# cwida/ALP

Measured on AMD Instinct MI355X. Metric: ALP fused decode (falp + patch) throughput, decoded doubles, higher is better.
Workload: dtype f64

## Files before the change

### alp_amd/csrc/init_kernels.hip

```cpp
#include <cstdlib>

#include "launch.hpp"
#include "rd_dictionary_order.hpp"
#include "search_device.hpp"

namespace alpgpu {

constexpr int kMaxSampledVectors = 9;
constexpr int kInitThreads       = 64 * kMaxSampledVectors;
#ifndef ALPGPU_INIT_ASYNC_WAVES
#define ALPGPU_INIT_ASYNC_WAVES 4
#endif
constexpr int kInitAsyncWaves        = ALPGPU_INIT_ASYNC_WAVES;
#ifndef ALPGPU_INIT_ASYNC_OCC
#define ALPGPU_INIT_ASYNC_OCC (ALPGPU_INIT_ASYNC_WAVES == 4 ? 5 : 8)
#endif
constexpr int kInitAsyncWavesPerSimd = ALPGPU_INIT_ASYNC_OCC;

__device__ __forceinline__ int wave_scan_max_i32(int v) {
	int t;
	t = __builtin_amdgcn_update_dpp(-1, v, 0x111, 0xf, 0xf, false), v = t > v ? t : v;
	t = __builtin_amdgcn_update_dpp(-1, v, 0x112, 0xf, 0xf, false), v = t > v ? t : v;
	t = __builtin_amdgcn_update_dpp(-1, v, 0x114, 0xf, 0xf, false), v = t > v ? t : v;
	t = __builtin_amdgcn_update_dpp(-1, v, 0x118, 0xf, 0xf, false), v = t > v ? t : v;
	t = __builtin_amdgcn_update_dpp(-1, v, 0x142, 0xa, 0xf, false), v = t > v ? t : v;
	t = __builtin_amdgcn_update_dpp(-1, v, 0x143, 0xc, 0xf, false), v = t > v ? t : v;
	return v;
}

constexpr int kMaxSamples = kMaxSampledVectors * 32;

struct __attribute__((aligned(16))) RdWaveScratch {
	uint32_t len[kMaxSamples];
	uint32_t hist[kMaxSamples + 8];
};

__device__ __forceinline__ uint32_t rd_left_of(uint32_t composite, int cut) { return (composite >> 16) >> (16 - cut); }

__device__ __forceinline__ void rd_build_runs(RdWaveScratch& W, uint32_t* first, const uint32_t* s_key, int n_smp, int cut, int lane) {
	for (int b = 0; b < kMaxSamples + 8; b += 64) {
		const int j = b + lane;
		if (j < kMaxSamples) {
			W.len[j] = 0u;
			if (first) { first[j] = 0xFFFFFFFFu; }
		}
		if (j < kMaxSamples + 8) { W.hist[j] = 0u; }
	}
	wave_lds_sync();
	int carry = 0;
	for (int b = 0; b < n_smp; b += 64) {
		const int      j     = b + lane;
		const bool     valid = j < n_smp;
		const uint32_t left  = valid ? rd_left_of(s_key[j], cut) : 0u;
		const uint32_t prev  = (valid && j > 0) ? rd_left_of(s_key[j - 1], cut) : ~left;
		const bool     head  = valid && (j == 0 || left != prev);
		int            st    = wave_scan_max_i32(head ? j : -1);
		st                   = st < 0 ? carry : st;
		if (valid) {
			atomicAdd(&W.len[st], 1u);
			if (first) { atomicMin(&first[st], s_key[j] & 0xFFFFu); }
		}
		carry = __builtin_amdgcn_readlane(st, 63);
	}
	wave_lds_sync();
}

template <bool ASYNC>
__device__ __forceinline__ void store_rowgroup_state(alpgpu_rowgroup_state* __restrict__ dst, const alpgpu_rowgroup_state& st) {
	if constexpr (!ASYNC) {
		*dst = st;
	} else {
		uint64_t w[4];
		__builtin_memcpy(w, &st, 32);
		w[1] = (w[1] & 0x00FFFFFFFFFFFFFFull) | (static_cast<uint64_t>(kStateReady) << 56);
		uint64_t* d64 = reinterpret_cast<uint64_t*>(dst);
		__hip_atomic_store(d64 + 0, w[0], __ATOMIC_RELAXED, __HIP_MEMORY_SCOPE_AGENT);
		__hip_atomic_store(d64 + 2, w[2], __ATOMIC_RELAXED, __HIP_MEMORY_SCOPE_AGENT);
		__hip_atomic_store(d64 + 3, w[3], __ATOMIC_RELAXED, __HIP_MEMORY_SCOPE_AGENT);
		asm volatile("s_waitcnt vmcnt(0)" ::: "memory");
		__hip_atomic_store(d64 + 1, w[1], __ATOMIC_RELAXED, __HIP_MEMORY_SCOPE_AGENT);
	}
}

constexpr int kInitAsyncTileWaves = 8;
template <bool ASYNC, int W, int BITS>
constexpr int init_waves_per_simd() {
	return !ASYNC ? 1 : (W == kInitAsyncWaves ? kInitAsyncWavesPerSimd : (W == kInitAsyncTileWaves ? (BITS == 32 ? 8 : 6) : 1));
}
template <class P, bool FROM_SAMPLES, int W, bool ASYNC>
__global__ __launch_bounds__(64 * W, (init_waves_per_simd<ASYNC, W, P::kBits>())) void k_rowgroup_init(const typename P::value_t* __restrict__ in, uint64_t n_vectors,
                                                          alpgpu_rowgroup_state* __restrict__ rgs, int force_rd,
                                                          uint16_t* __restrict__ rd_order, uint64_t rg_first, uint64_t rg_end, double* __restrict__ cut_est_out,
                                                          uint32_t adaptive_base) {
	static_assert(!ASYNC || !FROM_SAMPLES, "the persistent form gathers its own samples");
	static_assert(W >= 2 && W <= kMaxSampledVectors, "the scratch arrays are sized for 9 wavefronts; wavefront 0 and the order replay use two of them");
	__shared__ typename P::value_t smp[kMaxSampledVectors * 32];
	__shared__ uint32_t best_key[kMaxSampledVectors];
	__shared__ uint32_t      s_key[kMaxSamples];
	constexpr int kRdScratch = W > 4 ? W : 4;
#ifdef ALPGPU_EXPERIMENT_INIT_SMALL_LDS
	__shared__ RdWaveScratch s_rd[1];
#else
	__shared__ RdWaveScratch s_rd[kRdScratch];
#endif
	__shared__ uint32_t      s_first[kMaxSamples];
	__shared__ double        s_cut_est[17];
	__shared__ uint8_t       s_cut_ds[17];
	__shared__ int           s_best_cut;
	__shared__ int           s_scheme;
	__shared__ alpgpu_rowgroup_state s_state;

	const int      lane    = lane_id();
	const int      wave    = wave_in_wg();
	const int      tid     = static_cast<int>(threadIdx.x);
	(void)rg_end;
	uint32_t walkers = gridDim.x;
	if constexpr (ASYNC) {
		if (adaptive_base != 0 && adaptive_base < gridDim.x) {
			const bool     rd    = rgs[4 * lane].scheme == ALPGPU_SCHEME_ALP_RD;
			const bool     heavy = __builtin_popcountll(ballot64(rd)) >= 32;
			walkers              = heavy ? gridDim.x : adaptive_base;
			if (blockIdx.x >= walkers) { return; }
		}
	}
	for (uint64_t rg = rg_first + blockIdx.x; ASYNC ? rg < rg_end : rg == rg_first + blockIdx.x; rg += ASYNC ? walkers : 1u << 30) {
	if (ASYNC) { __syncthreads(); }
	int n_sv, n_smp, samples_size;
	if constexpr (FROM_SAMPLES) {
		n_smp        = static_cast<int>(n_vectors);
		n_sv         = (n_smp + 31) / 32;
		samples_size = n_smp < 32 ? n_smp : 32;
		for (int sv = wave; sv < n_sv; sv += W) {
			if (lane < 32) { smp[sv * 32 + lane] = in[288ull * blockIdx.x + sv * samples_size + (lane < samples_size ? lane : 0)]; }
		}
	} else {
		const uint64_t v_first = rg * kRowgroup;
		const int      nv      = static_cast<int>((n_vectors - v_first) < kRowgroup ? (n_vectors - v_first) : kRowgroup);
		n_sv                   = (nv + 11) / 12;
		n_smp                  = 32 * n_sv;
		samples_size           = 32;
		for (int sv = wave; sv < n_sv; sv += W) {
			if (lane < 32) { smp[sv * 32 + lane] = in[(v_first + 12ull * sv) * kVec + 32ull * lane]; }
		}
	}
	if (tid < kMaxSampledVectors) { best_key[tid] = 0xFFFFFFFFu; }
	__syncthreads();

	if (!force_rd) {
		constexpr int  kTail       = P::kNumCombos % 64;
		constexpr bool kTailOnSide = P::kBits == 32 && kTail > 0 && kTail <= 2;
		constexpr int  kRounds     = kTailOnSide ? P::kNumCombos / 64 : (P::kNumCombos + 63) / 64;
		constexpr int  kItemsPerSv = kRounds + (kTailOnSide ? 1 : 0);
#pragma unroll 1
		for (int item = wave; item < n_sv * kItemsPerSv; item += W) {
			const int sv = item / kItemsPerSv;
			const int r  = item - sv * kItemsPerSv;
			uint32_t  my_key = 0xFFFFFFFFu;
			if (kTailOnSide && r == kRounds) {
				const int  half   = lane >> 5, sidx = lane & 31;
				const int  c      = P::kNumCombos - kTail + (half < kTail ? half : 0);
				const bool active = half < kTail && sidx < samples_size;
				const typename P::Coef k = P::coef(P::combos().e[c], P::combos().f[c]);
				const float   v  = static_cast<float>(smp[sv * 32 + (sidx < samples_size ? sidx : 0)]);
				const int32_t q  = encode_value_f32(v, k.exp10, k.frac_f);
				const bool    ok = active & (decode_value_f32(q, k.fact, k.frac_e) == v);
				const uint64_t bal     = ballot64(ok);
				const int      non_exc = __builtin_popcount(static_cast<uint32_t>(half ? (bal >> 32) : bal));
				int32_t        mx = ok ? q : INT32_MIN, mn = ok ? q : INT32_MAX;
#define ALPGPU_MINMAX_STEP(CTRL, ROWS)                                                                                  \
	{                                                                                                                   \
		const int32_t omx = __builtin_amdgcn_update_dpp(mx, mx, CTRL, ROWS, 0xf, false);                                \
		const int32_t omn = __builtin_amdgcn_update_dpp(mn, mn, CTRL, ROWS, 0xf, false);                                \
		mx                = omx > mx ? omx : mx;                                                                        \
		mn                = omn < mn ? omn : mn;                                                                        \
	}
				ALPGPU_MINMAX_STEP(0x111, 0xf)
				ALPGPU_MINMAX_STEP(0x112, 0xf)
				ALPGPU_MINMAX_STEP(0x114, 0xf)
				ALPGPU_MINMAX_STEP(0x118, 0xf)
				ALPGPU_MINMAX_STEP(0x142, 0xa)
#undef ALPGPU_MINMAX_STEP
				if (sidx == 31 && half < kTail && non_exc >= 2) {
					const uint32_t size = static_cast<uint32_t>(samples_size) * static_cast<uint32_t>(P::bits(mx, mn)) +
					                      static_cast<uint32_t>(samples_size - non_exc) * (P::kExcBits + 16u);
					my_key              = (size << 8) | static_cast<uint32_t>(c);
				}
			} else {
				const int c = lane + 64 * r;
				if (c < P::kNumCombos) {
					const typename P::Coef k = P::coef(P::combos().e[c], P::combos().f[c]);
					typename P::Acc        acc;
					P::start(acc);
					if constexpr (P::kBits == 64) {
						int s = 0;
						for (; s + 4 <= samples_size; s += 4) {
							P::step(acc, smp[sv * 32 + s], k);
							P::step(acc, smp[sv * 32 + s + 1], k);
							P::step(acc, smp[sv * 32 + s + 2], k);
							P::step(acc, smp[sv * 32 + s + 3], k);
						}
						for (; s < samples_size; ++s) { P::step(acc, smp[sv * 32 + s], k); }
					} else {
#pragma unroll 4
						for (int s = 0; s < samples_size; ++s) { P::step(acc, smp[sv * 32 + s], k); }
					}
					P::finish(acc);
					const int     non_exc = acc.non_exc;
					const int64_t mx = acc.mx, mn = acc.mn;
					if (non_exc >= 2) {
						const uint32_t size = static_cast<uint32_t>(samples_size) * static_cast<uint32_t>(P::bits(mx, mn)) +
						                      static_cast<uint32_t>(samples_size - non_exc) * (P::kExcBits + 16u);
						my_key              = (size << 8) | static_cast<uint32_t>(c);
					}
				}
			}
			my_key = wave_min_u32(my_key);
			if (lane == 0 && my_key != 0xFFFFFFFFu) { atomicMin(&best_key[sv], my_key); }
		}
	}
	__syncthreads();

	if (tid == 0) {
		uint32_t best_size = static_cast<uint32_t>(samples_size) * (P::kExcBits + 16u) + static_cast<uint32_t>(samples_size) * P::kExcBits;
		int      ce[kMaxSampledVectors], cf[kMaxSampledVectors], cn[kMaxSampledVectors];
		int      n_c = 0;
		for (int w = 0; w < n_sv; ++w) {
			int e = 0, f = 0;
			if (best_key[w] != 0xFFFFFFFFu) {
				const int      c    = static_cast<int>(best_key[w] & 0xFFu);
				const uint32_t size = best_key[w] >> 8;
				e                   = P::combos().e[c];
				f                   = P::combos().f[c];
				best_size           = size < best_size ? size : best_size;
			}
			int hit = -1;
			for (int i = 0; i < n_c; ++i) {
				if (ce[i] == e && cf[i] == f) { hit = i; }
			}
			if (hit < 0) {
				ce[n_c] = e, cf[n_c] = f, cn[n_c] = 1;
				++n_c;
			} else {
				++cn[hit];
			}
		}
		alpgpu_rowgroup_state st;
		st.k = 0;
		for (int i = 0; i < 10; ++i) { st.combos[i] = 0; }
		st.rd_rbw = st.rd_lbw = st.rd_dict_size = st.pad = 0;
		for (int i = 0; i < 8; ++i) { st.rd_dict[i] = 0; }
		if (force_rd || best_size >= P::kRdThreshold) {
			st.scheme = ALPGPU_SCHEME_ALP_RD;
		} else {
			st.scheme = ALPGPU_SCHEME_ALP;
			for (int i = 1; i < n_c; ++i) {
				const int e = ce[i], f = cf[i], n = cn[i];
				int       j = i - 1;
				while (j >= 0 && (n > cn[j] || (n == cn[j] && e > ce[j]) || (n == cn[j] && e == ce[j] && f > cf[j]))) {
					ce[j + 1] = ce[j], cf[j + 1] = cf[j], cn[j + 1] = cn[j];
					--j;
				}
				ce[j + 1] = e, cf[j + 1] = f, cn[j + 1] = n;
			}
			const int k = n_c < 5 ? n_c : 5;
			st.k        = static_cast<uint8_t>(k);
#pragma unroll
			for (int i = 0; i < 5; ++i) {
				st.combos[2 * i]     = i < k ? static_cast<uint8_t>(ce[i]) : 0;
				st.combos[2 * i + 1] = i < k ? static_cast<uint8_t>(cf[i]) : 0;
			}
		}
		s_scheme = st.scheme;
		if (st.scheme != ALPGPU_SCHEME_ALP_RD) {
			store_rowgroup_state<ASYNC>(rgs + rg, st);
			if (rd_order) { rd_order[rg * ALPGPU_RD_ORDER_STRIDE] = 0; }
		} else {
			s_state = st;
		}
	}
	__syncthreads();
	if (s_scheme != ALPGPU_SCHEME_ALP_RD) { continue; }
#ifdef ALPGPU_EXPERIMENT_INIT_SMALL_LDS
	continue;
#endif

	uint32_t* s_unsorted = reinterpret_cast<uint32_t*>(&s_rd[0]);
	static_assert(sizeof(RdWaveScratch) >= kMaxSamples * sizeof(uint32_t), "scratch reuse");
	static_assert(kMaxSamples % 4 == 0, "the rank loop reads four keys at a time");
	constexpr int kSortSlots = (kMaxSamples + 64 * W - 1) / (64 * W);
	for (int t = tid; t < kMaxSamples; t += 64 * W) {
		uint32_t c = 0xFFFFFFFFu;
		if (t < n_smp) { c = (static_cast<uint32_t>(P::pattern(smp[32 * (t / samples_size) + (t % samples_size)]) >> (P::kBits - 16)) << 16) | static_cast<uint32_t>(t); }
		s_unsorted[t] = c;
	}
	__syncthreads();
	uint32_t my_key[kSortSlots];
	int      my_rank[kSortSlots];
#pragma unroll
	for (int u = 0; u < kSortSlots; ++u) {
		const int t = tid + u * 64 * W;
		my_key[u]   = 0;
		my_rank[u]  = 0;
		if (t < n_smp) {
			my_key[u]          = s_unsorted[t];
			const u32x4* quads = reinterpret_cast<const u32x4*>(s_unsorted);
			const int    n_q   = (n_smp + 3) / 4;
			for (int q = 0; q < n_q; ++q) {
				const u32x4 k = quads[q];
				my_rank[u] += (k[0] < my_key[u] ? 1 : 0) + (k[1] < my_key[u] ? 1 : 0) + (k[2] < my_key[u] ? 1 : 0) + (k[3] < my_key[u] ? 1 : 0);
			}
		}
	}
	__syncthreads();
#pragma unroll
	for (int u = 0; u < kSortSlots; ++u) {
		if (tid + u * 64 * W < n_smp) { s_key[my_rank[u]] = my_key[u]; }
	}
	__syncthreads();

#ifdef ALPGPU_EXPERIMENT_RD_STOP_AFTER_SORT
	continue;
#endif
	RdWaveScratch& WS = s_rd[wave];
#ifdef ALPGPU_EXPERIMENT_RD_ONE_CUT
	const int forced_cut = 12;
#else
	const int forced_cut = (force_rd & 0x100) ? (force_rd & 0xFF) : 0;
#endif
	for (int cut = wave + 1; cut <= 16; cut += W) {
		const int rbw = P::kBits - cut;
		if (forced_cut != 0 && cut != forced_cut) {
			if (lane == 0) {
				s_cut_est[cut] = 1.7976931348623157e308;
				s_cut_ds[cut]  = 0;
			}
			continue;
		}
		rd_build_runs(WS, nullptr, s_key, n_smp, cut, lane);
		int distinct = 0;
		for (int b = 0; b < n_smp; b += 64) {
			const int      j = b + lane;
			const uint32_t L = j < n_smp ? WS.len[j] : 0u;
			if (L) { atomicAdd(&WS.hist[L], 1u); }
			distinct += __builtin_popcountll(__ballot(L != 0));
		}
		wave_lds_sync();
		uint32_t covered = 0;
		int      taken   = 0;
		for (int top = n_smp; top >= 1 && taken < 8; top -= 64) {
			const int      cval = top - lane;
			const uint32_t h    = cval >= 1 ? WS.hist[cval] : 0u;
			const uint32_t inc    = wave_scan_add_u32(h);
			const uint32_t before = static_cast<uint32_t>(taken) + inc - h;
			const uint32_t after  = static_cast<uint32_t>(taken) + inc;
			const uint32_t mine   = (after < 8u ? after : 8u) - (before < 8u ? before : 8u);
			const uint32_t part   = wave_scan_add_u32(mine * static_cast<uint32_t>(cval > 0 ? cval : 0));
			covered += static_cast<uint32_t>(__builtin_amdgcn_readlane(static_cast<int>(part), 63));
			taken += __builtin_amdgcn_readlane(static_cast<int>(inc), 63);
		}
		const uint32_t excs = static_cast<uint32_t>(n_smp) - covered;
		const int      ds   = distinct < 8 ? distinct : 8;
		const int      lbw  = ds <= 2 ? 1 : (ds <= 4 ? 2 : 3);
		if (lane == 0) {
			s_cut_est[cut] = static_cast<double>(rbw + lbw) + static_cast<double>(excs * 32u) / static_cast<double>(n_smp);
			s_cut_ds[cut]  = static_cast<uint8_t>(ds);
		}
		wave_lds_sync();
	}
	__syncthreads();
	if (tid == 0) {
		double best = 1.7976931348623157e308;
		int    bc   = 1;
		for (int cut = 1; cut <= 16; ++cut) {
			if (s_cut_est[cut] < best) {
				best = s_cut_est[cut];
				bc   = cut;
			}
		}
		s_best_cut = bc;
		if (cut_est_out != nullptr) { cut_est_out[blockIdx.x] = best; }
	}
	__syncthreads();
	if (wave == 0) {
		static_assert(sizeof(RdOrderLds) <= (kRdScratch - 1) * sizeof(RdWaveScratch), "order replay arrays alias s_rd[1..]");
		RdOrderLds& s_order = *reinterpret_cast<RdOrderLds*>(&s_rd[1]);
		const int best_cut = s_best_cut;
		const int rbw      = P::kBits - best_cut;
		const int ds       = s_cut_ds[best_cut];
		rd_build_runs(WS, s_first, s_key, n_smp, best_cut, lane);
		int distinct = 0;
		for (int b = 0; b < n_smp; b += 64) {
			const int      j    = b + lane;
			const bool     head = j < n_smp && WS.len[j] != 0;
			const uint64_t hb   = __ballot(head);
			if (head) { s_order.sorted[distinct + __builtin_popcountll(hb & ((1ull << lane) - 1ull))] = s_first[j]; }
			distinct += __builtin_popcountll(hb);
		}
		wave_lds_sync();
		for (int b = 0; b < n_smp; b += 64) {
			const int      j   = b + lane;
			const uint32_t L   = j < n_smp ? WS.len[j] : 0u;
			const uint32_t fo  = j < n_smp ? s_first[j] : 0u;
			int            ord = 0;
			for (int g = 0; g < distinct; ++g) { ord += s_order.sorted[g] < fo ? 1 : 0; }
			if (L != 0) {
				s_order.okey[ord] = rd_left_of(s_key[j], best_cut);
				s_order.ocnt[ord] = L;
			}
		}
		wave_lds_sync();
#ifndef ALPGPU_EXPERIMENT_SKIP_RD_ORDER
		if (lane == 0) { rd_reference_order(s_order, distinct); }
#endif
		wave_lds_sync();
		if (rd_order) {
			uint16_t* o = rd_order + rg * ALPGPU_RD_ORDER_STRIDE;
			for (int i = lane; i < distinct; i += 64) { o[1 + i] = static_cast<uint16_t>(s_order.sorted[i] & 0xFFFFu); }
			if (lane == 0) { o[0] = static_cast<uint16_t>(distinct); }
		}
		if constexpr (ASYNC) {
			if (rd_order) {
				__builtin_amdgcn_fence(__ATOMIC_RELEASE, "agent");
				asm volatile("s_waitcnt vmcnt(0)" ::: "memory");
			}
		}
		if (lane == 0) {
			const int             lbw = ds <= 2 ? 1 : (ds <= 4 ? 2 : 3);
			alpgpu_rowgroup_state st  = s_state;
			st.rd_rbw                 = static_cast<uint8_t>(rbw);
			st.rd_lbw                 = static_cast<uint8_t>(lbw);
			st.rd_dict_size           = static_cast<uint8_t>(ds);
#pragma unroll
			for (int i = 0; i < 8; ++i) { st.rd_dict[i] = i < ds ? static_cast<uint16_t>(s_order.sorted[i] & 0xFFFFu) : 0; }
			store_rowgroup_state<ASYNC>(rgs + rg, st);
		}
	}
	}
}

int launch_rowgroup_init(hipStream_t stream, const double* d_in, uint64_t n_vectors, alpgpu_rowgroup_state* d_rgs, uint16_t* d_rd_order, uint64_t rg_first,
                         uint64_t rg_count) {
	const uint64_t n_rg = (n_vectors + kRowgroup - 1) / kRowgroup;
	if (rg_first >= n_rg) { return ALPGPU_OK; }
	if (rg_count == 0 || rg_first + rg_count > n_rg) { rg_count = n_rg - rg_first; }
	hipLaunchKernelGGL((k_rowgroup_init<PrecF64, false, kMaxSampledVectors, false>), dim3(static_cast<unsigned>(rg_count)), dim3(kInitThreads), 0, stream, d_in,
	                   n_vectors, d_rgs, 0, d_rd_order, rg_first, rg_first + rg_count, static_cast<double*>(nullptr), 0u);
	return hipGetLastError() == hipSuccess ? ALPGPU_OK : ALPGPU_ERR_HIP;
}

template <class P>
static int launch_rowgroup_init_async_t(hipStream_t stream, const typename P::value_t* d_in, uint64_t n_vectors, alpgpu_rowgroup_state* d_rgs, uint16_t* d_rd_order,
                                        uint64_t rg_first, uint64_t rg_count, int grid, bool tile_shaped, uint32_t adaptive_base = 0) {
	if (rg_count == 0) { return ALPGPU_OK; }
	const uint64_t g = rg_count < static_cast<uint64_t>(grid) ? rg_count : static_cast<uint64_t>(grid);
	if (g == rg_count) {
		hipLaunchKernelGGL((k_rowgroup_init<P, false, kMaxSampledVectors, true>), dim3(static_cast<unsigned>(g)), dim3(kInitThreads), 0, stream, d_in, n_vectors, d_rgs, 0,
		                   d_rd_order, rg_first, rg_first + rg_count, static_cast<double*>(nullptr), 0u);
	} else if (tile_shaped) {
		hipLaunchKernelGGL((k_rowgroup_init<P, false, kInitAsyncTileWaves, true>), dim3(static_cast<unsigned>(g)), dim3(64 * kInitAsyncTileWaves), 0, stream, d_in, n_vectors,
		                   d_rgs, 0, d_rd_order, rg_first, rg_first + rg_count, static_cast<double*>(nullptr), adaptive_base);
	} else {
		hipLaunchKernelGGL((k_rowgroup_init<P, false, kInitAsyncWaves, true>), dim3(static_cast<unsigned>(g)), dim3(64 * kInitAsyncWaves), 0, stream, d_in, n_vectors, d_rgs,
		                   0, d_rd_order, rg_first, rg_first + rg_count, static_cast<double*>(nullptr), adaptive_base);
	}
	return hipGetLastError() == hipSuccess ? ALPGPU_OK : ALPGPU_ERR_HIP;
}
int launch_rowgroup_init_async(hipStream_t stream, const double* d_in, uint64_t n_vectors, alpgpu_rowgroup_state* d_rgs, uint16_t* d_rd_order, uint64_t rg_first,
                               uint64_t rg_count, int grid, bool tile_shaped, uint32_t adaptive_base) {
	return launch_rowgroup_init_async_t<PrecF64>(stream, d_in, n_vectors, d_rgs, d_rd_order, rg_first, rg_count, grid, tile_shaped, adaptive_base);
}
int launch_rowgroup_init_async_f32(hipStream_t stream, const float* d_in, uint64_t n_vectors, alpgpu_rowgroup_state* d_rgs, uint16_t* d_rd_order, uint64_t rg_first,
                                   uint64_t rg_count, int grid) {
	static const bool tile = std::getenv("ALPGPU_F32_SEARCH_TILE") != nullptr;
	return launch_rowgroup_init_async_t<PrecF32>(stream, d_in, n_vectors, d_rgs, d_rd_order, rg_first, rg_count, grid, tile);
}

int launch_state_from_samples(hipStream_t stream, const double* d_samples, uint32_t n_samples, alpgpu_rowgroup_state* d_state, int force_rd, double* d_cut_estimate) {
	hipLaunchKernelGGL((k_rowgroup_init<PrecF64, true, kMaxSampledVectors, false>), dim3(1), dim3(kInitThreads), 0, stream, d_samples, static_cast<uint64_t>(n_samples),
	                   d_state, force_rd, static_cast<uint16_t*>(nullptr), 0ull, 1ull, d_cut_estimate, 0u);
	return hipGetLastError() == hipSuccess ? ALPGPU_OK : ALPGPU_ERR_HIP;
}

int launch_rowgroup_init_f32(hipStream_t stream, const float* d_in, uint64_t n_vectors, alpgpu_rowgroup_state* d_rgs, uint16_t* d_rd_order,
                             uint64_t rg_first, uint64_t rg_count) {
	const uint64_t n_rg = (n_vectors + kRowgroup - 1) / kRowgroup;
	if (rg_first >= n_rg) { return ALPGPU_OK; }
	if (rg_count == 0 || rg_first + rg_count > n_rg) { rg_count = n_rg - rg_first; }
	hipLaunchKernelGGL((k_rowgroup_init<PrecF32, false, kMaxSampledVectors, false>), dim3(static_cast<unsigned>(rg_count)), dim3(kInitThreads), 0, stream, d_in,
	                   n_vectors, d_rgs, 0, d_rd_order, rg_first, rg_first + rg_count, static_cast<double*>(nullptr), 0u);
	return hipGetLastError() == hipSuccess ? ALPGPU_OK : ALPGPU_ERR_HIP;
}

int launch_state_from_samples_f32(hipStream_t stream, const float* d_samples, uint32_t n_samples, alpgpu_rowgroup_state* d_state, int force_rd, double* d_cut_estimate) {
	hipLaunchKernelGGL((k_rowgroup_init<PrecF32, true, kMaxSampledVectors, false>), dim3(1), dim3(kInitThreads), 0, stream, d_samples, static_cast<uint64_t>(n_samples),
	                   d_state, force_rd, static_cast<uint16_t*>(nullptr), 0ull, 1ull, d_cut_estimate, 0u);
	return hipGetLastError() == hipSuccess ? ALPGPU_OK : ALPGPU_ERR_HIP;
}

}
```

Before: 4461.

## Compute ALP-RD run lengths in registers via ballots instead of LDS atomics

Replaces the per-wave LDS scratch (run lengths plus histogram built with LDS atomics) with register-resident sorted keys and ballot bitmasks that give run heads and lengths directly. The top-8 coverage is found by eight wave-wide max reductions instead of a histogram scan. The dictionary-order replay now scatters first-occurrence indices instead of doing an O(distinct) rank loop per lane. LDS use shrinks to a union, which could allow higher occupancy in the init kernel. This is an init-path change whose effect on the fused decode metric may be small. The rewritten first-occurrence and order logic risks subtle correctness differences.

```diff
diff --git a/alp_amd/csrc/init_kernels.hip b/alp_amd/csrc/init_kernels.hip
--- a/alp_amd/csrc/init_kernels.hip
+++ b/alp_amd/csrc/init_kernels.hip
@@ -30,39 +30,62 @@
 
 constexpr int kMaxSamples = kMaxSampledVectors * 32;
 
-struct __attribute__((aligned(16))) RdWaveScratch {
-	uint32_t len[kMaxSamples];
-	uint32_t hist[kMaxSamples + 8];
+__device__ __forceinline__ uint32_t rd_left_of(uint32_t composite, int cut) { return (composite >> 16) >> (16 - cut); }
+
+constexpr int kKeyChunks = (kMaxSamples + 63) / 64;
+struct RdSortedKeys {
+	uint32_t key[kKeyChunks], prev[kKeyChunks];
 };
-
-__device__ __forceinline__ uint32_t rd_left_of(uint32_t composite, int cut) { return (composite >> 16) >> (16 - cut); }
-
-__device__ __forceinline__ void rd_build_runs(RdWaveScratch& W, uint32_t* first, const uint32_t* s_key, int n_smp, int cut, int lane) {
-	for (int b = 0; b < kMaxSamples + 8; b += 64) {
-		const int j = b + lane;
-		if (j < kMaxSamples) {
-			W.len[j] = 0u;
-			if (first) { first[j] = 0xFFFFFFFFu; }
-		}
-		if (j < kMaxSamples + 8) { W.hist[j] = 0u; }
-	}
-	wave_lds_sync();
-	int carry = 0;
-	for (int b = 0; b < n_smp; b += 64) {
-		const int      j     = b + lane;
-		const bool     valid = j < n_smp;
-		const uint32_t left  = valid ? rd_left_of(s_key[j], cut) : 0u;
-		const uint32_t prev  = (valid && j > 0) ? rd_left_of(s_key[j - 1], cut) : ~left;
-		const bool     head  = valid && (j == 0 || left != prev);
-		int            st    = wave_scan_max_i32(head ? j : -1);
-		st                   = st < 0 ? carry : st;
-		if (valid) {
-			atomicAdd(&W.len[st], 1u);
-			if (first) { atomicMin(&first[st], s_key[j] & 0xFFFFu); }
-		}
-		carry = __builtin_amdgcn_readlane(st, 63);
-	}
-	wave_lds_sync();
+__device__ __forceinline__ void rd_load_keys(RdSortedKeys& K, const uint32_t* s_key, int n_smp, int lane) {
+#pragma unroll
+	for (int c = 0; c < kKeyChunks; ++c) {
+		const int j = 64 * c + lane;
+		K.key[c]    = j < n_smp ? s_key[j] : 0xFFFFFFFFu;
+		K.prev[c]   = (j > 0 && j < n_smp) ? s_key[j - 1] : 0u;
+	}
+}
+
+struct RdRuns {
+	uint64_t head[kKeyChunks];
+	uint32_t len[kKeyChunks];
+	int      distinct;
+};
+__device__ __forceinline__ void rd_runs(RdRuns& R, const RdSortedKeys& K, int n_smp, int cut, int lane) {
+	R.distinct = 0;
+#pragma unroll
+	for (int c = 0; c < kKeyChunks; ++c) {
+		const int j = 64 * c + lane;
+		R.head[c]   = ballot64((j < n_smp) & ((j == 0) | (rd_left_of(K.key[c], cut) != rd_left_of(K.prev[c], cut))));
+		R.distinct += __builtin_popcountll(R.head[c]);
+	}
+	int next_start = n_smp;
+#pragma unroll
+	for (int c = kKeyChunks - 1; c >= 0; --c) {
+		const uint64_t above = R.head[c] & ~((2ull << lane) - 1ull);
+		const int      next  = above ? 64 * c + __builtin_ctzll(above) : next_start;
+		R.len[c]             = ((R.head[c] >> lane) & 1ull) ? static_cast<uint32_t>(next - (64 * c + lane)) : 0u;
+		if (R.head[c]) { next_start = 64 * c + __builtin_ctzll(R.head[c]); }
+	}
+}
+
+__device__ __forceinline__ uint32_t rd_top8_mass(const RdRuns& R, int n_smp, int lane) {
+	if (R.distinct <= 8) { return static_cast<uint32_t>(n_smp); }
+	static_assert(kMaxSamples < 512, "positions take 9 bits");
+	uint32_t u[kKeyChunks];
+#pragma unroll
+	for (int c = 0; c < kKeyChunks; ++c) { u[c] = R.len[c] ? (R.len[c] << 9) | static_cast<uint32_t>(64 * c + lane) : 0u; }
+	uint32_t covered = 0;
+#pragma unroll
+	for (int i = 0; i < 8; ++i) {
+		uint32_t m = u[0];
+#pragma unroll
+		for (int c = 1; c < kKeyChunks; ++c) { m = u[c] > m ? u[c] : m; }
+		const uint32_t top = static_cast<uint32_t>(__builtin_amdgcn_readlane(wave_scan_max_i32(static_cast<int>(m)), 63));
+		covered += top >> 9;
+#pragma unroll
+		for (int c = 0; c < kKeyChunks; ++c) { u[c] = u[c] == top ? 0u : u[c]; }
+	}
+	return covered;
 }
 
 template <bool ASYNC>
@@ -93,16 +116,14 @@
                                                           uint16_t* __restrict__ rd_order, uint64_t rg_first, uint64_t rg_end, double* __restrict__ cut_est_out,
                                                           uint32_t adaptive_base) {
 	static_assert(!ASYNC || !FROM_SAMPLES, "the persistent form gathers its own samples");
-	static_assert(W >= 2 && W <= kMaxSampledVectors, "the scratch arrays are sized for 9 wavefronts; wavefront 0 and the order replay use two of them");
+	static_assert(W >= 2 && W <= kMaxSampledVectors, "best_key and the sample arrays are sized for 9 sampled vectors");
 	__shared__ typename P::value_t smp[kMaxSampledVectors * 32];
 	__shared__ uint32_t best_key[kMaxSampledVectors];
 	__shared__ uint32_t      s_key[kMaxSamples];
-	constexpr int kRdScratch = W > 4 ? W : 4;
-#ifdef ALPGPU_EXPERIMENT_INIT_SMALL_LDS
-	__shared__ RdWaveScratch s_rd[1];
-#else
-	__shared__ RdWaveScratch s_rd[kRdScratch];
-#endif
+	__shared__ union {
+		uint32_t   unsorted[kMaxSamples];
+		RdOrderLds order;
+	} s_rdx;
 	__shared__ uint32_t      s_first[kMaxSamples];
 	__shared__ double        s_cut_est[17];
 	__shared__ uint8_t       s_cut_ds[17];
@@ -280,12 +301,8 @@
 	}
 	__syncthreads();
 	if (s_scheme != ALPGPU_SCHEME_ALP_RD) { continue; }
-#ifdef ALPGPU_EXPERIMENT_INIT_SMALL_LDS
-	continue;
-#endif
-
-	uint32_t* s_unsorted = reinterpret_cast<uint32_t*>(&s_rd[0]);
-	static_assert(sizeof(RdWaveScratch) >= kMaxSamples * sizeof(uint32_t), "scratch reuse");
+
+	uint32_t* s_unsorted = s_rdx.unsorted;
 	static_assert(kMaxSamples % 4 == 0, "the rank loop reads four keys at a time");
 	constexpr int kSortSlots = (kMaxSamples + 64 * W - 1) / (64 * W);
 	for (int t = tid; t < kMaxSamples; t += 64 * W) {
@@ -321,7 +338,8 @@
 #ifdef ALPGPU_EXPERIMENT_RD_STOP_AFTER_SORT
 	continue;
 #endif
-	RdWaveScratch& WS = s_rd[wave];
+	RdSortedKeys K;
+	rd_load_keys(K, s_key, n_smp, lane);
 #ifdef ALPGPU_EXPERIMENT_RD_ONE_CUT
 	const int forced_cut = 12;
 #else
@@ -336,36 +354,15 @@
 			}
 			continue;
 		}
-		rd_build_runs(WS, nullptr, s_key, n_smp, cut, lane);
-		int distinct = 0;
-		for (int b = 0; b < n_smp; b += 64) {
-			const int      j = b + lane;
-			const uint32_t L = j < n_smp ? WS.len[j] : 0u;
-			if (L) { atomicAdd(&WS.hist[L], 1u); }
-			distinct += __builtin_popcountll(__ballot(L != 0));
-		}
-		wave_lds_sync();
-		uint32_t covered = 0;
-		int      taken   = 0;
-		for (int top = n_smp; top >= 1 && taken < 8; top -= 64) {
-			const int      cval = top - lane;
-			const uint32_t h    = cval >= 1 ? WS.hist[cval] : 0u;
-			const uint32_t inc    = wave_scan_add_u32(h);
-			const uint32_t before = static_cast<uint32_t>(taken) + inc - h;
-			const uint32_t after  = static_cast<uint32_t>(taken) + inc;
-			const uint32_t mine   = (after < 8u ? after : 8u) - (before < 8u ? before : 8u);
-			const uint32_t part   = wave_scan_add_u32(mine * static_cast<uint32_t>(cval > 0 ? cval : 0));
-			covered += static_cast<uint32_t>(__builtin_amdgcn_readlane(static_cast<int>(part), 63));
-			taken += __builtin_amdgcn_readlane(static_cast<int>(inc), 63);
-		}
-		const uint32_t excs = static_cast<uint32_t>(n_smp) - covered;
-		const int      ds   = distinct < 8 ? distinct : 8;
+		RdRuns R;
+		rd_runs(R, K, n_smp, cut, lane);
+		const uint32_t excs = static_cast<uint32_t>(n_smp) - rd_top8_mass(R, n_smp, lane);
+		const int      ds   = R.distinct < 8 ? R.distinct : 8;
 		const int      lbw  = ds <= 2 ? 1 : (ds <= 4 ? 2 : 3);
 		if (lane == 0) {
 			s_cut_est[cut] = static_cast<double>(rbw + lbw) + static_cast<double>(excs * 32u) / static_cast<double>(n_smp);
 			s_cut_ds[cut]  = static_cast<uint8_t>(ds);
 		}
-		wave_lds_sync();
 	}
 	__syncthreads();
 	if (tid == 0) {
@@ -382,31 +379,53 @@
 	}
 	__syncthreads();
 	if (wave == 0) {
-		static_assert(sizeof(RdOrderLds) <= (kRdScratch - 1) * sizeof(RdWaveScratch), "order replay arrays alias s_rd[1..]");
-		RdOrderLds& s_order = *reinterpret_cast<RdOrderLds*>(&s_rd[1]);
+		RdOrderLds& s_order = s_rdx.order;
 		const int best_cut = s_best_cut;
 		const int rbw      = P::kBits - best_cut;
 		const int ds       = s_cut_ds[best_cut];
-		rd_build_runs(WS, s_first, s_key, n_smp, best_cut, lane);
-		int distinct = 0;
-		for (int b = 0; b < n_smp; b += 64) {
-			const int      j    = b + lane;
-			const bool     head = j < n_smp && WS.len[j] != 0;
-			const uint64_t hb   = __ballot(head);
-			if (head) { s_order.sorted[distinct + __builtin_popcountll(hb & ((1ull << lane) - 1ull))] = s_first[j]; }
-			distinct += __builtin_popcountll(hb);
+		RdRuns    R;
+		rd_runs(R, K, n_smp, best_cut, lane);
+		const int distinct = R.distinct;
+		int prev_start = 0;
+#pragma unroll
+		for (int c = 0; c < kKeyChunks; ++c) {
+			const int      j    = 64 * c + lane;
+			const uint64_t upto = R.head[c] & ((2ull << lane) - 1ull);
+			const int      st   = upto ? 64 * c + 63 - __builtin_clzll(upto) : prev_start;
+			if (st == j && j < n_smp) { s_first[j] = K.key[c] & 0xFFFFu; }
+			if (R.head[c]) { prev_start = 64 * c + 63 - __builtin_clzll(R.head[c]); }
 		}
 		wave_lds_sync();
-		for (int b = 0; b < n_smp; b += 64) {
-			const int      j   = b + lane;
-			const uint32_t L   = j < n_smp ? WS.len[j] : 0u;
-			const uint32_t fo  = j < n_smp ? s_first[j] : 0u;
-			int            ord = 0;
-			for (int g = 0; g < distinct; ++g) { ord += s_order.sorted[g] < fo ? 1 : 0; }
-			if (L != 0) {
-				s_order.okey[ord] = rd_left_of(s_key[j], best_cut);
-				s_order.ocnt[ord] = L;
-			}
+		prev_start = 0;
+#pragma unroll
+		for (int c = 0; c < kKeyChunks; ++c) {
+			const int      j    = 64 * c + lane;
+			const uint64_t upto = R.head[c] & ((2ull << lane) - 1ull);
+			const int      st   = upto ? 64 * c + 63 - __builtin_clzll(upto) : prev_start;
+			if (st != j && j < n_smp && (K.key[c] >> 16) != (K.prev[c] >> 16)) { atomicMin(&s_first[st], K.key[c] & 0xFFFFu); }
+			if (R.head[c]) { prev_start = 64 * c + 63 - __builtin_clzll(R.head[c]); }
+		}
+#pragma unroll
+		for (int c = 0; c < kKeyChunks; ++c) {
+			if (64 * c + lane < n_smp) { s_order.sorted[64 * c + lane] = 0u; }
+		}
+		wave_lds_sync();
+#pragma unroll
+		for (int c = 0; c < kKeyChunks; ++c) {
+			if (R.len[c] != 0u) { s_order.sorted[s_first[64 * c + lane]] = (R.len[c] << 16) | rd_left_of(K.key[c], best_cut); }
+		}
+		wave_lds_sync();
+		uint32_t n_out = 0;
+#pragma unroll
+		for (int c = 0; c < kKeyChunks; ++c) {
+			const uint32_t v   = 64 * c + lane < n_smp ? s_order.sorted[64 * c + lane] : 0u;
+			const uint64_t has = ballot64(v != 0u);
+			if (v != 0u) {
+				const uint32_t o = mbcnt64(has, n_out);
+				s_order.okey[o] = v & 0xFFFFu;
+				s_order.ocnt[o] = v >> 16;
+			}
+			n_out += static_cast<uint32_t>(__builtin_popcountll(has));
 		}
 		wave_lds_sync();
 #ifndef ALPGPU_EXPERIMENT_SKIP_RD_ORDER
```

Measured after the change: 4461 (median of 6 runs). No clear change (-0.0%).
